# SingleRust/single-algebra

Hardware: AMD Instinct MI355X
Metric: sparse_pca_fit_transform_algorithmic_throughput (higher is better)
Workload: dtype f32

## Files before the change

single-algebra_amd/csrc/tiled_build.hip:

```cpp
#include <algorithm>
#include <cmath>
#include <cstdio>
#include <cstdlib>
#include <cstring>
#include <vector>

#include <rocprim/rocprim.hpp>

#include "kernels.h"
#include "quad_format.h"
#include "spmm_dq.h"

namespace sapca {
namespace k {

namespace {

__device__ __forceinline__ void divmod_small(int c, int d, float inv, int& q, int& r) {
  q = (int)((float)c * inv);
  r = c - q * d;
  if (r < 0) { r += d; --q; }
  if (r >= d) { r -= d; ++q; }
}

__global__ void __launch_bounds__(256)
tile_hist_kernel(const int64_t* __restrict__ ptr, const int32_t* __restrict__ idx, int64_t rows, int nct, float inv_nct,
                 int32_t* __restrict__ seg) {
  extern __shared__ uint32_t hist_all[];
  const int wave = threadIdx.x / WAVE, lane = threadIdx.x & (WAVE - 1);
  uint32_t* hist = hist_all + (size_t)wave * nct;
  for (int64_t r = (int64_t)blockIdx.x * 4 + wave; r < rows; r += (int64_t)gridDim.x * 4) {
    for (int t = lane; t < nct; t += WAVE) hist[t] = 0;
    __builtin_amdgcn_wave_barrier();
    const int64_t e0 = ptr[r], e1 = ptr[r + 1];
    for (int64_t eb = e0 + lane; eb < e1; eb += 8 * WAVE) {
      int c[8];
#pragma unroll
      for (int u = 0; u < 8; ++u) c[u] = eb + u * WAVE < e1 ? idx[eb + u * WAVE] : -1;
#pragma unroll
      for (int u = 0; u < 8; ++u)
        if (c[u] >= 0) {
          int q, t;
          divmod_small(c[u], nct, inv_nct, q, t);
          atomicAdd(&hist[t], 1u);
        }
    }
    __builtin_amdgcn_wave_barrier();
    uint32_t carry = 0;
    int32_t* out = seg + r * (nct + 1);
    for (int t0 = 0; t0 < nct; t0 += WAVE) {
      const int t = t0 + lane;
      const uint32_t v = t < nct ? hist[t] : 0u;
      uint32_t x = v;
#pragma unroll
      for (int off = 1; off < WAVE; off <<= 1) {
        const uint32_t y = __shfl_up(x, off);
        if (lane >= off) x += y;
      }
      if (t < nct) out[t] = (int32_t)(carry + x - v);
      carry += __shfl(x, WAVE - 1);
    }
    if (lane == 0) out[nct] = (int32_t)carry;
    __builtin_amdgcn_wave_barrier();
  }
}

constexpr int QC_TILES = 8;
__global__ void __launch_bounds__(Q_BLOCK_QUADS)
quad_count_kernel(const int32_t* __restrict__ seg, const int32_t* __restrict__ blk_row0, const uint32_t* __restrict__ perm,
                  int nct, uint16_t* __restrict__ steps, uint32_t* __restrict__ quad_off, uint32_t* __restrict__ wave_off,
                  int64_t* __restrict__ chunk_size, const uint16_t* __restrict__ cnt16 = nullptr, int64_t cnt_stride = 0,
                  int64_t* __restrict__ raw_size = nullptr) {
  __shared__ uint32_t scan[Q_BLOCK_QUADS];
  __shared__ uint32_t wave_total[Q_BLOCK_QUADS / WAVE], raw_part[Q_BLOCK_QUADS / WAVE];
  const int groups = (nct + QC_TILES - 1) / QC_TILES;
  const int rb = blockIdx.x / groups, ct0 = (blockIdx.x % groups) * QC_TILES;
  const int row0 = blk_row0[rb], nrows = blk_row0[rb + 1] - row0;
  const int nquads = (nrows + 3) / 4;
  const int q = threadIdx.x, lane = q & (WAVE - 1);
  int len[4][QC_TILES];
#pragma unroll
  for (int g = 0; g < 4; ++g) {
    const int lr = 4 * q + g;
    const bool have = lr < nrows;
    const int64_t r = have ? (perm ? (int64_t)perm[row0 + lr] : (int64_t)row0 + lr) : 0;
    if (cnt16) {
#pragma unroll
      for (int j = 0; j < QC_TILES; ++j) len[g][j] = (have && ct0 + j < nct) ? (int)cnt16[(int64_t)(ct0 + j) * cnt_stride + r] : 0;
    } else {
      int bound[QC_TILES + 1];
#pragma unroll
      for (int j = 0; j <= QC_TILES; ++j) bound[j] = (have && ct0 + j <= nct) ? seg[r * (nct + 1) + ct0 + j] : 0;
#pragma unroll
      for (int j = 0; j < QC_TILES; ++j) len[g][j] = (have && ct0 + j < nct) ? bound[j + 1] - bound[j] : 0;
    }
  }
#pragma unroll
  for (int j = 0; j < QC_TILES; ++j) {
    const int ct = ct0 + j;
    if (ct >= nct) break;
    const int64_t chunk = (int64_t)rb * nct + ct;
    const int longest = max(max(len[0][j], len[1][j]), max(len[2][j], len[3][j]));
    int raw = len[0][j] + len[1][j] + len[2][j] + len[3][j];
    const int qmax = q_steps(longest);
    const uint32_t padded = (uint32_t)qmax * 4u;
    steps[chunk * Q_BLOCK_QUADS + q] = (uint16_t)qmax;
    uint32_t inc = padded;
#pragma unroll
    for (int off = 1; off < WAVE; off <<= 1) {
      const uint32_t y = __shfl_up(inc, off);
      if (lane >= off) inc += y;
    }
#pragma unroll
    for (int off = WAVE / 2; off > 0; off >>= 1) raw += __shfl_xor(raw, off);
    __syncthreads();
    if (lane == WAVE - 1) wave_total[q / WAVE] = inc;
    if (lane == 0) raw_part[q / WAVE] = (uint32_t)raw;
    __syncthreads();
    for (int w = 0; w < q / WAVE; ++w) inc += wave_total[w];
    scan[q] = inc;
    __syncthreads();
    if (quad_off && q < nquads) quad_off[((int64_t)rb * Q_BLOCK_QUADS + q) * nct + ct] = inc - padded;
    if (q < QWAVES) {
      const int first_quad = q_first(q, nquads);
      wave_off[chunk * QWAVES + q] = first_quad > 0 ? scan[first_quad - 1] : 0u;
    }
    if (q == Q_BLOCK_QUADS - 1) {
      chunk_size[chunk] = inc;
      if (raw_size) {
        uint32_t total = 0;
        for (int w = 0; w < Q_BLOCK_QUADS / WAVE; ++w) total += raw_part[w];
        raw_size[chunk] = total;
      }
    }
  }
}

template <typename VT>
__global__ void __launch_bounds__(256)
quad_fill_kernel(const int64_t* __restrict__ ptr, const int32_t* __restrict__ idx, const VT* __restrict__ val,
                 int64_t rows, const int32_t* __restrict__ blk_row0, const uint32_t* __restrict__ perm, int nrb, int nct,
                 float inv_nct, int ldp_bytes, const int64_t* __restrict__ chunk_off, const uint32_t* __restrict__ quad_off,
                 typename EntOf<VT>::type* __restrict__ ent) {
  typedef typename EntOf<VT>::type E;
  extern __shared__ uint32_t cnt_all[];
  const int wave = threadIdx.x / WAVE, lane = threadIdx.x & (WAVE - 1);
  uint32_t* cnt = cnt_all + (size_t)wave * nct;
  const int64_t sp = (int64_t)blockIdx.x * 4 + wave;
  if (sp >= rows) return;
  const int64_t r = perm ? (int64_t)perm[sp] : sp;
  int lo = 0, hi = nrb;
  while (hi - lo > 1) {
    const int mid = (lo + hi) >> 1;
    if ((int64_t)blk_row0[mid] <= sp) lo = mid; else hi = mid;
  }
  const int rb = lo;
  const int lr = (int)(sp - blk_row0[rb]);
  const int qd = lr >> 2;
  const uint32_t g = (uint32_t)(lr & 3);
  const int64_t* __restrict__ coff = chunk_off + (int64_t)rb * nct;
  const uint32_t* __restrict__ qoff = quad_off + ((int64_t)rb * Q_BLOCK_QUADS + qd) * nct;
  const int64_t block_base = coff[0];
  for (int t = lane; t < nct; t += WAVE) cnt[t] = (uint32_t)(coff[t] - block_base) + qoff[t] + g;
  __builtin_amdgcn_wave_barrier();
  const int64_t e0 = ptr[r], e1 = ptr[r + 1];
  E* __restrict__ out = ent + block_base;
  for (int64_t eb = e0; eb < e1; eb += 8 * WAVE) {
    int c[8];
    VT v[8];
#pragma unroll
    for (int u = 0; u < 8; ++u) {
      const int64_t e = eb + u * WAVE + lane;
      c[u] = e < e1 ? idx[e] : -1;
      v[u] = e < e1 ? val[e] : (VT)0;
    }
#pragma unroll
    for (int u = 0; u < 8; ++u) {
      if (c[u] >= 0) {
        int i, t;
        divmod_small(c[u], nct, inv_nct, i, t);
        E x = E();
        x.off = (uint32_t)i * (uint32_t)ldp_bytes;
        x.val = v[u];
        out[atomicAdd(&cnt[t], 4u)] = x;
      }
      __builtin_amdgcn_wave_barrier();
    }
  }
}

constexpr int QF_CAP_MIN = 4096, QF_CAP_MAX = 6144;
template <typename VT>
__device__ __forceinline__ void quad_fill_staged_one(int qi, uint32_t* qf_lds, const int64_t* __restrict__ ptr, const int32_t* __restrict__ idx,
                                                     const VT* __restrict__ val, const int32_t* __restrict__ seg,
                                                     const int32_t* __restrict__ blk_row0, const uint32_t* __restrict__ perm, int nct, int cap,
                                                     float inv_nct, int ldp_bytes, const int64_t* __restrict__ chunk_off,
                                                     const uint32_t* __restrict__ quad_off, typename EntOf<VT>::type* __restrict__ ent) {
  typedef typename EntOf<VT>::type E;
  constexpr int EW = (int)sizeof(E) / 4;
  E* stage = reinterpret_cast<E*>(qf_lds);
  int64_t* gofs = reinterpret_cast<int64_t*>(qf_lds + EW * cap);
  uint32_t* lofs = qf_lds + EW * cap + 2 * nct;
  uint32_t* cnt_all = lofs + nct + 1;
  const int rb = qi / Q_BLOCK_QUADS, qd = qi % Q_BLOCK_QUADS;
  const int row0 = blk_row0[rb], nrows = blk_row0[rb + 1] - row0;
  if (4 * qd >= nrows) return;
  const int wave = threadIdx.x / WAVE, lane = threadIdx.x & (WAVE - 1);
  const int qrows = min(4, nrows - 4 * qd);
  const int64_t s0 = (int64_t)row0 + 4 * qd;
  int64_t rowof[4];
#pragma unroll
  for (int g = 0; g < 4; ++g) rowof[g] = g < qrows ? (perm ? (int64_t)perm[s0 + g] : s0 + g) : 0;
  const int64_t* __restrict__ coff = chunk_off + (int64_t)rb * nct;
  const uint32_t* __restrict__ qoff = quad_off + ((int64_t)rb * Q_BLOCK_QUADS + qd) * nct;
  for (int t = threadIdx.x; t < nct; t += 256) {
    int mx = 0;
    for (int g = 0; g < qrows; ++g) {
      const int32_t* sg = seg + rowof[g] * (nct + 1);
      mx = max(mx, sg[t + 1] - sg[t]);
    }
    lofs[t + 1] = (uint32_t)q_steps(mx) * 4u;
    gofs[t] = coff[t] + (int64_t)qoff[t];
    for (int g = 0; g < 4; ++g) cnt_all[g * nct + t] = 0;
  }
  if (threadIdx.x == 0) lofs[0] = 0;
  __syncthreads();
  if (wave == 0) {
    uint32_t carry = 0;
    for (int t0 = 0; t0 < nct; t0 += WAVE) {
      const int t = t0 + lane;
      const uint32_t v = t < nct ? lofs[t + 1] : 0u;
      uint32_t x = v;
#pragma unroll
      for (int off = 1; off < WAVE; off <<= 1) {
        const uint32_t y = __shfl_up(x, off);
        if (lane >= off) x += y;
      }
      if (t < nct) lofs[t + 1] = carry + x;
      carry += __shfl(x, WAVE - 1);
    }
  }
  __syncthreads();
  const uint32_t total = lofs[nct];
  const bool staged = total <= (uint32_t)cap;
  if (staged) {
    uint64_t* z = reinterpret_cast<uint64_t*>(stage);
    for (uint32_t i = threadIdx.x; i < total * (EW / 2); i += 256) z[i] = 0;
  } else {
    if (wave < qrows) {
      const int32_t* sg = seg + rowof[wave] * (nct + 1);
      for (int t = lane; t < nct; t += WAVE) {
        const uint32_t steps = (lofs[t + 1] - lofs[t]) / 4u;
        E* dst = ent + gofs[t];
        for (uint32_t k = (uint32_t)(sg[t + 1] - sg[t]); k < steps; ++k) dst[k * 4u + wave] = E();
      }
    } else {
      for (int t = lane; t < nct; t += WAVE) {
        const uint32_t steps = (lofs[t + 1] - lofs[t]) / 4u;
        E* dst = ent + gofs[t];
        for (uint32_t k = 0; k < steps; ++k) dst[k * 4u + wave] = E();
      }
    }
  }
  __syncthreads();
  if (wave < qrows) {
    const int64_t r = rowof[wave];
    const int64_t e0 = ptr[r], e1 = ptr[r + 1];
    uint32_t* cnt = cnt_all + (size_t)wave * nct;
    for (int64_t eb = e0; eb < e1; eb += 8 * WAVE) {
      int c[8];
      VT v[8];
#pragma unroll
      for (int u = 0; u < 8; ++u) {
        const int64_t e = eb + u * WAVE + lane;
        c[u] = e < e1 ? idx[e] : -1;
        v[u] = e < e1 ? val[e] : (VT)0;
      }
#pragma unroll
      for (int u = 0; u < 8; ++u) {
        if (c[u] >= 0) {
          int i, t;
          divmod_small(c[u], nct, inv_nct, i, t);
          E x = E();
          x.off = (uint32_t)i * (uint32_t)ldp_bytes;
          x.val = v[u];
          const uint32_t k = atomicAdd(&cnt[t], 1u);
          if (staged) stage[lofs[t] + k * 4u + (uint32_t)wave] = x;
          else ent[gofs[t] + k * 4u + (uint32_t)wave] = x;
        }
        __builtin_amdgcn_wave_barrier();
      }
    }
  }
  if (!staged) return;
  __syncthreads();
  for (int t = wave; t < nct; t += 4) {
    const uint32_t lo = lofs[t], n = lofs[t + 1] - lo;
    E* dst = ent + gofs[t];
    for (uint32_t j = lane; j < n; j += WAVE) dst[j] = stage[lo + j];
  }
}

template <typename VT>
__global__ void __launch_bounds__(256)
quad_fill_staged_kernel(const int64_t* __restrict__ ptr, const int32_t* __restrict__ idx, const VT* __restrict__ val,
                        const int32_t* __restrict__ seg, const int32_t* __restrict__ blk_row0,
                        const uint32_t* __restrict__ perm, int nct, int cap, float inv_nct,
                        int ldp_bytes, const int64_t* __restrict__ chunk_off, const uint32_t* __restrict__ quad_off,
                        typename EntOf<VT>::type* __restrict__ ent, int nquads_all) {
  extern __shared__ __attribute__((aligned(16))) uint32_t qf_lds[];
  for (int qi = blockIdx.x; qi < nquads_all; qi += gridDim.x) {
    quad_fill_staged_one<VT>(qi, qf_lds, ptr, idx, val, seg, blk_row0, perm, nct, cap, inv_nct, ldp_bytes, chunk_off, quad_off, ent);
    __syncthreads();
  }
}

__global__ void tile_index_mod_kernel(const int64_t* __restrict__ ptr, const int32_t* __restrict__ idx,
                                      const uint64_t* __restrict__ packed, int64_t rows, int nct, float inv_nct,
                                      int32_t* __restrict__ seg) {
  const int64_t total = rows * (int64_t)(nct + 1);
  int64_t o = (int64_t)blockIdx.x * blockDim.x + threadIdx.x;
  const int64_t stride = (int64_t)gridDim.x * blockDim.x;
  for (; o < total; o += stride) {
    const int64_t r = o / (nct + 1);
    const int t = (int)(o - r * (nct + 1));
    const int64_t e0 = ptr[r], e1 = ptr[r + 1];
    int64_t lo = e0, hi = e1;
    while (lo < hi) {
      const int64_t mid = (lo + hi) >> 1;
      int q, tm;
      divmod_small(packed ? (int)(packed[mid] >> 32) : idx[mid], nct, inv_nct, q, tm);
      if (tm < t) lo = mid + 1; else hi = mid;
    }
    seg[o] = (int32_t)(lo - e0);
  }
}

__global__ void at_stats_index_kernel(const int64_t* __restrict__ ptr, const uint64_t* __restrict__ packed, int64_t rows,
                                      int nct, float inv_nct, double* __restrict__ sum, double* __restrict__ sumsq,
                                      int32_t* __restrict__ seg) {
  const int lane = threadIdx.x & (WAVE - 1);
  const int64_t wave = ((int64_t)blockIdx.x * blockDim.x + threadIdx.x) / WAVE;
  const int64_t nwaves = (int64_t)gridDim.x * blockDim.x / WAVE;
  for (int64_t r = wave; r < rows; r += nwaves) {
    const int64_t e0 = ptr[r], e1 = ptr[r + 1];
    int32_t* sg = seg + r * (nct + 1);
    double a = 0, b = 0;
    int carry = -1;
    for (int64_t eb = e0; eb < e1; eb += WAVE) {
      const int64_t e = eb + lane;
      const bool valid = e < e1;
      int t = nct;
      if (valid) {
        const uint64_t pv = packed[e];
        const double v = (double)__uint_as_float((uint32_t)pv);
        a += v;
        b += v * v;
        int q;
        divmod_small((int)(pv >> 32), nct, inv_nct, q, t);
      }
      int tprev = __shfl_up(t, 1);
      if (lane == 0) tprev = carry;
      if (valid || e == e1)
        for (int tt = tprev + 1; tt <= t; ++tt) sg[tt] = (int32_t)(e - e0);
      carry = __shfl(t, WAVE - 1);
    }
    if (((e1 - e0) & (WAVE - 1)) == 0)
      for (int tt = carry + 1 + lane; tt <= nct; tt += WAVE) sg[tt] = (int32_t)(e1 - e0);
#pragma unroll
    for (int off = WAVE / 2; off > 0; off >>= 1) {
      a += __shfl_xor(a, off);
      b += __shfl_xor(b, off);
    }
    if (lane == 0) {
      sum[r] = a;
      if (sumsq) sumsq[r] = b;
    }
  }
}

__global__ void row_len_iota_kernel(const int64_t* __restrict__ ptr, int64_t rows, uint32_t* __restrict__ len,
                                    uint32_t* __restrict__ iota) {
  const int64_t r = (int64_t)blockIdx.x * blockDim.x + threadIdx.x;
  if (r < rows) {
    len[r] = (uint32_t)(ptr[r + 1] - ptr[r]);
    iota[r] = (uint32_t)r;
  }
}

__global__ void __launch_bounds__(256)
natural_quad_slots_kernel(const int64_t* __restrict__ ptr, int64_t rows, unsigned long long* __restrict__ out) {
  __shared__ unsigned long long red[4];
  unsigned long long acc = 0;
  const int64_t nq = (rows + 3) / 4;
  for (int64_t qd = (int64_t)blockIdx.x * blockDim.x + threadIdx.x; qd < nq; qd += (int64_t)gridDim.x * blockDim.x) {
    int64_t mx = 0;
    for (int g = 0; g < 4 && 4 * qd + g < rows; ++g) mx = max(mx, ptr[4 * qd + g + 1] - ptr[4 * qd + g]);
    acc += (unsigned long long)(4 * mx);
  }
#pragma unroll
  for (int off = WAVE / 2; off > 0; off >>= 1) acc += __shfl_xor(acc, off);
  if ((threadIdx.x & (WAVE - 1)) == 0) red[threadIdx.x / WAVE] = acc;
  __syncthreads();
  if (threadIdx.x == 0) atomicAdd(out, red[0] + red[1] + red[2] + red[3]);
}

template <bool SEG_LDS, typename VT = float>
__global__ void __launch_bounds__(256)
quad_fill_runs_kernel(const int64_t* __restrict__ ptr, const int32_t* __restrict__ idx, const VT* __restrict__ val,
                      const uint64_t* __restrict__ packed, const int32_t* __restrict__ seg, const int32_t* __restrict__ blk_row0,
                      const uint32_t* __restrict__ perm, int nct, float inv_nct, int ldp_bytes,
                      const int64_t* __restrict__ chunk_off, const uint32_t* __restrict__ quad_off,
                      typename EntOf<VT>::type* __restrict__ ent) {
  typedef typename EntOf<VT>::type Ent;
  extern __shared__ int32_t sg_lds[];
  const int rb = blockIdx.x / Q_BLOCK_QUADS, qd = blockIdx.x % Q_BLOCK_QUADS;
  const int row0 = blk_row0[rb], nrows = blk_row0[rb + 1] - row0;
  if (4 * qd >= nrows) return;
  const int wave = threadIdx.x / WAVE, lane = threadIdx.x & (WAVE - 1);
  const int qrows = min(4, nrows - 4 * qd);
  const int64_t s0q = (int64_t)row0 + 4 * qd;
  if (SEG_LDS) {
    for (int i = threadIdx.x; i < 4 * (nct + 1); i += 256) {
      const int g = i / (nct + 1);
      const int64_t rg = g < qrows ? (perm ? (int64_t)perm[s0q + g] : s0q + g) : 0;
      sg_lds[i] = g < qrows ? seg[rg * (nct + 1) + (i - g * (nct + 1))] : 0;
    }
    __syncthreads();
  }
  const int g = lane & 3, k0 = lane >> 2;
  const int64_t myrow = g < qrows ? (perm ? (int64_t)perm[s0q + g] : s0q + g) : -1;
  const int64_t base = myrow >= 0 ? ptr[myrow] : 0;
  const int32_t* mysg = SEG_LDS ? sg_lds + g * (nct + 1) : seg + (myrow >= 0 ? myrow : 0) * (nct + 1);
  const int64_t* __restrict__ coff = chunk_off + (int64_t)rb * nct;
  const uint32_t* __restrict__ qoff = quad_off + ((int64_t)rb * Q_BLOCK_QUADS + qd) * nct;
  int s_nx = 0, e_nx = 0;
  int64_t d_nx = 0;
  if (!SEG_LDS && wave < nct) {
    s_nx = myrow >= 0 ? mysg[wave] : 0;
    e_nx = myrow >= 0 ? mysg[wave + 1] : 0;
    d_nx = coff[wave] + qoff[wave];
  }
  for (int t = wave; t < nct; t += 4) {
    int s0, len;
    Ent* dst;
    if (SEG_LDS) {
      s0 = mysg[t];
      len = mysg[t + 1] - s0;
      dst = ent + coff[t] + qoff[t];
    } else {
      s0 = s_nx;
      len = e_nx - s_nx;
      dst = ent + d_nx;
      if (t + 4 < nct) {
        s_nx = myrow >= 0 ? mysg[t + 4] : 0;
        e_nx = myrow >= 0 ? mysg[t + 5] : 0;
        d_nx = coff[t + 4] + qoff[t + 4];
      }
    }
    int qmax = max(len, __shfl_xor(len, 1));
    qmax = q_steps(max(qmax, __shfl_xor(qmax, 2)));
    for (int k = k0; k < qmax; k += 16) {
      Ent x{};
      if (k < len) {
        const int64_t e = base + s0 + k;
        int c;
        if constexpr (sizeof(VT) == 4) {
          if (packed) {
            const uint64_t pv = packed[e];
            c = (int)(pv >> 32);
            x.val = __uint_as_float((uint32_t)pv);
          } else {
            c = idx[e];
            x.val = val[e];
          }
        } else {
          c = idx[e];
          x.val = val[e];
        }
        int i, tm;
        divmod_small(c, nct, inv_nct, i, tm);
        x.off = (uint32_t)i * (uint32_t)ldp_bytes;
      }
      dst[k * 4 + g] = x;
    }
  }
}

template <int PER, bool HAS_B>
__global__ void __launch_bounds__(1024)
small_scan_kernel(int64_t* __restrict__ a, int64_t* __restrict__ b, int64_t count, int64_t* __restrict__ out_max_total) {
  __shared__ int64_t wsum[2][16], wmax[16];
  const int tid = threadIdx.x, lane = tid & (WAVE - 1), wave = tid / WAVE;
  int64_t carry_a = 0, carry_b = 0, m = 0;
  for (int64_t base = 0; base < count; base += 1024 * PER) {
    const int64_t lo = min(count, base + (int64_t)tid * PER), hi = min(count, lo + PER);
    int64_t sa = 0, sb = 0, mx = 0;
    int64_t ra_[PER], rb_[HAS_B ? PER : 1];
#pragma unroll
    for (int u = 0; u < PER; ++u) {
      ra_[u] = lo + u < hi ? a[lo + u] : 0;
      if constexpr (HAS_B) rb_[u] = lo + u < hi ? b[lo + u] : 0;
    }
#pragma unroll
    for (int u = 0; u < PER; ++u) {
      sa += ra_[u];
      mx = max(mx, ra_[u]);
      if constexpr (HAS_B) sb += rb_[u];
    }
    int64_t ia = sa, ib = sb;
#pragma unroll
    for (int off = 1; off < WAVE; off <<= 1) {
      const int64_t ya = __shfl_up(ia, off), yb = __shfl_up(ib, off);
      if (lane >= off) { ia += ya; ib += yb; }
    }
#pragma unroll
    for (int off = WAVE / 2; off > 0; off >>= 1) mx = max(mx, __shfl_xor(mx, off));
    __syncthreads();
    if (lane == WAVE - 1) { wsum[0][wave] = ia; wsum[1][wave] = ib; }
    if (lane == 0) wmax[wave] = mx;
    __syncthreads();
    int64_t ra = carry_a + ia - sa, rb = carry_b + ib - sb, ta = 0, tb = 0;
#pragma unroll 2
    for (int w = 0; w < 16; ++w) {
      if (w < wave) { ra += wsum[0][w]; rb += wsum[1][w]; }
      ta += wsum[0][w];
      tb += wsum[1][w];
      m = max(m, wmax[w]);
    }
    carry_a += ta;
    carry_b += tb;
#pragma unroll
    for (int u = 0; u < PER; ++u) {
      if (lo + u < hi) {
        a[lo + u] = ra;
        if constexpr (HAS_B) b[lo + u] = rb;
      }
      ra += ra_[u];
      if constexpr (HAS_B) rb += rb_[u];
    }
  }
  if (tid == 0) {
    a[count] = carry_a;
    if (HAS_B && b) b[count] = carry_b;
    if (out_max_total) { out_max_total[0] = m; out_max_total[1] = carry_a; }
  }
}

void launch_small_scan(int64_t* a, int64_t* b, int64_t count, int64_t* out_max_total, hipStream_t s) {
  const int64_t per = (count + 1023) / 1024;
  if (b && per <= 8) hipLaunchKernelGGL((small_scan_kernel<8, true>), dim3(1), dim3(1024), 0, s, a, b, count, out_max_total);
  else if (b) hipLaunchKernelGGL((small_scan_kernel<16, true>), dim3(1), dim3(1024), 0, s, a, b, count, out_max_total);
  else hipLaunchKernelGGL((small_scan_kernel<24, false>), dim3(1), dim3(1024), 0, s, a, b, count, out_max_total);
}

constexpr int ATD_MAX_COLS = 65536;
constexpr int ATD_THREADS = 1024;
constexpr int ATD_MASK_WORDS = 10;

constexpr int ATD_HIST_THREADS = 512;
constexpr int ATD_HIST_THREADS_WIDE = 1024;

__global__ void __launch_bounds__(ATD_HIST_THREADS_WIDE)
atd_hist_kernel(const int64_t* __restrict__ ptr, const int32_t* __restrict__ idx, int64_t m, int nct, int tc, int64_t n2,
                uint16_t* __restrict__ cnt16, float blk_scale, int nrb, uint32_t* __restrict__ bnd, int64_t* __restrict__ disorder,
                unsigned long long* __restrict__ slots_to_clear) {
  if (blockIdx.x == 0 && threadIdx.x == 0 && slots_to_clear) *slots_to_clear = 0ull;
  extern __shared__ uint32_t atd_h32[];
  const int t = blockIdx.x;
  const int nw = (int)(n2 / 2);
  const int nthreads = (int)blockDim.x, nwaves = nthreads / WAVE;
  for (int i = threadIdx.x; i < nw; i += nthreads) atd_h32[i] = 0u;
  __syncthreads();
  const int wave = threadIdx.x / WAVE, lane = threadIdx.x & (WAVE - 1);
  int64_t r = (int64_t)t + (int64_t)wave * nct;
  int64_t e0 = (wave < tc && r < m) ? ptr[r] : 0, e1 = (wave < tc && r < m) ? ptr[r + 1] : 0;
  for (int i = wave; i < tc; i += nwaves) {
    if (r >= m) {
      if (bnd)
        for (int j = lane; j <= nrb; j += WAVE) bnd[((int64_t)t * tc + i) * (nrb + 1) + j] = 0u;
      continue;
    }
    const int64_t rn = r + (int64_t)nwaves * nct;
    const bool more = i + nwaves < tc && rn < m;
    const int64_t n0 = more ? ptr[rn] : 0, n1 = more ? ptr[rn + 1] : 0;
    int lastb = -1;
    uint32_t* __restrict__ bnd_row = bnd ? bnd + ((int64_t)t * tc + i) * (nrb + 1) : nullptr;
    const int64_t row_e0 = e0;
    for (int64_t base = e0; base < e1; base += 8 * WAVE) {
      const int64_t eb = base + lane;
      int c[8];
#pragma unroll
      for (int u = 0; u < 8; ++u) c[u] = eb + u * WAVE < e1 ? idx[eb + u * WAVE] : -1;
      if (bnd) {
#pragma unroll
        for (int u = 0; u < 8; ++u) {
          const bool valid = c[u] >= 0;
          const unsigned long long valids = __ballot(valid);
          if (valids == 0ull) break;
          const int b = (int)((float)max(c[u], 0) * blk_scale);
          const int up = __builtin_amdgcn_update_dpp(0, b, 0x138, 0xf, 0xf, false);
          const int prev = lane == 0 ? lastb : up;
          if (valid && b != prev)
            for (int j = prev + 1; j <= b; ++j) bnd_row[j] = (uint32_t)(eb + u * WAVE - row_e0);
          if (valid && b < prev) *disorder = 1;
          lastb = __builtin_amdgcn_readlane(b, __builtin_popcountll(valids) - 1);
        }
      }
#pragma unroll
      for (int u = 0; u < 8; ++u)
        if (c[u] >= 0) atomicAdd(&atd_h32[c[u] >> 1], 1u << (16 * (c[u] & 1)));
    }
    if (bnd)
      for (int j = lastb + 1 + lane; j <= nrb; j += WAVE) bnd_row[j] = (uint32_t)(e1 - row_e0);
    r = rn;
    e0 = n0;
    e1 = n1;
  }
  __syncthreads();
  uint32_t* out = reinterpret_cast<uint32_t*>(cnt16 + (int64_t)t * n2);
  for (int i = threadIdx.x; i < nw; i += nthreads) out[i] = atd_h32[i];
}

__global__ void __launch_bounds__(1024)
atd_rowlen_kernel(const uint16_t* __restrict__ cnt16, int64_t n, int64_t n2, int nct, int64_t* __restrict__ len,
                  unsigned long long* __restrict__ natural_slots) {
  __shared__ uint32_t part[16][64];
  const int lane = threadIdx.x & 63, grp = threadIdx.x >> 6;
  const int64_t c = (int64_t)blockIdx.x * 64 + lane;
  const int per = (nct + 15) / 16;
  uint32_t a = 0;
  if (c < n) {
    const int t1 = min(nct, (grp + 1) * per);
    int t = grp * per;
    for (; t + 8 <= t1; t += 8) {
      uint32_t v[8];
#pragma unroll
      for (int u = 0; u < 8; ++u) v[u] = cnt16[(int64_t)(t + u) * n2 + c];
#pragma unroll
      for (int u = 0; u < 8; ++u) a += v[u];
    }
    for (; t < t1; ++t) a += cnt16[(int64_t)t * n2 + c];
  }
  part[grp][lane] = a;
  __syncthreads();
  if (grp == 0) {
    int64_t total = 0;
    if (c < n)
      for (int g = 0; g < 16; ++g) total += part[g][lane];
    if (c <= n) len[c] = total;
    if (natural_slots) {
      int64_t mx = max(total, __shfl_xor(total, 1));
      mx = max(mx, __shfl_xor(mx, 2));
      unsigned long long acc = (lane & 3) == 0 ? (unsigned long long)(4 * mx) : 0ull;
#pragma unroll
      for (int off = WAVE / 2; off > 0; off >>= 1) acc += __shfl_xor(acc, off);
      if (lane == 0 && acc) atomicAdd(natural_slots, acc);
    }
  }
}

__global__ void atd_colmap_kernel(const int32_t* __restrict__ blk, int nrb, const uint32_t* __restrict__ perm, int64_t rows,
                                  uint32_t* __restrict__ colmap) {
  const int64_t sp = (int64_t)blockIdx.x * blockDim.x + threadIdx.x;
  if (sp >= rows) return;
  int lo = 0, hi = nrb;
  while (lo + 1 < hi) {
    const int mid = (lo + hi) >> 1;
    if ((int64_t)blk[mid] <= sp) lo = mid; else hi = mid;
  }
  const int64_t row = perm ? (int64_t)perm[sp] : sp;
  colmap[row] = ((uint32_t)lo << 10) | (uint32_t)(sp - blk[lo]);
}

__global__ void __launch_bounds__(256)
atd_scatter_kernel(const int64_t* __restrict__ ptr, const int32_t* __restrict__ idx, const float* __restrict__ val, int64_t m, int nct,
                   int tc, const uint32_t* __restrict__ colmap, const int64_t* __restrict__ bucket_off, uint32_t* __restrict__ cursor,
                   uint2* __restrict__ bucket) {
  const int lane = threadIdx.x & (WAVE - 1);
  const int xcd = blockIdx.x & 7;
  const int64_t wave = (int64_t)(blockIdx.x >> 3) * (blockDim.x / WAVE) + threadIdx.x / WAVE;
  const int64_t nwaves = (int64_t)(gridDim.x >> 3) * (blockDim.x / WAVE);
  const int tiles_x = (nct - xcd + 7) / 8;
  const int64_t items = (int64_t)tiles_x * tc;
  constexpr int UB = 10;
  for (int64_t item = wave; item < items; item += nwaves) {
    const int i = (int)(item / tiles_x), t = xcd + 8 * (int)(item - (int64_t)i * tiles_x);
    const int64_t r = (int64_t)t + (int64_t)i * nct;
    if (r >= m) continue;
    const int64_t e1 = ptr[r + 1];
    for (int64_t eb = ptr[r]; eb < e1; eb += UB * WAVE) {
      int cc[UB];
      uint32_t cmv[UB];
      float vv[UB];
      int64_t base[UB];
      int mine[UB];
#pragma unroll
      for (int u = 0; u < UB; ++u) {
        const int64_t e = eb + u * WAVE + lane;
        cc[u] = e < e1 ? idx[e] : -1;
        vv[u] = e < e1 ? val[e] : 0.f;
      }
#pragma unroll
      for (int u = 0; u < UB; ++u) cmv[u] = cc[u] >= 0 ? colmap[cc[u]] : 0xffffffffu;
#pragma unroll
      for (int u = 0; u < UB; ++u) {
        const uint32_t rb = cmv[u] >> 10;
        const uint32_t prev = __shfl_up(rb, 1);
        const bool valid = cc[u] >= 0;
        const bool leader = valid && (lane == 0 || rb != prev);
        const unsigned long long leaders = __ballot(leader), valids = __ballot(valid);
        const unsigned long long upto = leaders & ((2ull << lane) - 1ull);
        mine[u] = upto ? 63 - __builtin_clzll(upto) : 0;
        base[u] = 0;
        if (leader) {
          const unsigned long long above = leaders & ~((2ull << lane) - 1ull);
          const int next = above ? __builtin_ctzll(above) : __builtin_popcountll(valids);
          const int64_t b = (int64_t)rb * nct + t;
          base[u] = bucket_off[b] + (int64_t)atomicAdd(&cursor[b], (uint32_t)(next - lane));
        }
      }
#pragma unroll
      for (int u = 0; u < UB; ++u) {
        const int64_t b0 = __shfl(base[u], mine[u]);
        if (cc[u] >= 0)
          bucket[b0 + (lane - mine[u])] = make_uint2(((cmv[u] & 1023u) << 9) | (uint32_t)i, __float_as_uint(vv[u]));
      }
    }
  }
}

constexpr int ATD_STAGE_ENT = 4096;

template <bool GATHER>
__global__ void __launch_bounds__(ATD_THREADS, 8)
atd_fill_kernel(const uint2* __restrict__ bucket, const int64_t* __restrict__ bucket_off, const int32_t* __restrict__ blk_row0,
                const uint32_t* __restrict__ perm, int nct, int ldp_bytes, const int64_t* __restrict__ chunk_off,
                const uint32_t* __restrict__ quad_off, const uint16_t* __restrict__ steps, Ent* __restrict__ ent,
                double* __restrict__ psum, double* __restrict__ psq, int64_t n,
                const int32_t* __restrict__ a_idx, const float* __restrict__ a_val, const uint32_t* __restrict__ bnd,
                const int64_t* __restrict__ a_ptr, int64_t a_rows, int tc, int nrb_all) {
  constexpr int MASK_WORDS_ALL = QBLOCK_ROWS * ATD_MASK_WORDS;
  __shared__ __attribute__((aligned(16))) uint32_t pool[MASK_WORDS_ALL + 2 * ATD_STAGE_ENT];
  uint32_t* mask = pool;
  Ent* stage = reinterpret_cast<Ent*>(pool + MASK_WORDS_ALL);
  __shared__ uint32_t qoff_s[Q_BLOCK_QUADS + 1];
  __shared__ uint32_t wtot[Q_BLOCK_QUADS / WAVE];
  __shared__ uint16_t len_s[QBLOCK_ROWS];
  __shared__ int64_t run_lo[GATHER ? 32 * ATD_MASK_WORDS : 1];
  __shared__ uint32_t run_pre[GATHER ? 32 * ATD_MASK_WORDS + 1 : 1];
  __shared__ uint32_t rtot[GATHER ? 32 * ATD_MASK_WORDS / WAVE : 1];
  int rb, t;
  if constexpr (GATHER) {
    const int xcd = blockIdx.x & 7, j = blockIdx.x >> 3;
    t = xcd + 8 * (j / nrb_all);
    rb = j % nrb_all;
    if (t >= nct) return;
  } else {
    rb = (int)(blockIdx.x / nct);
    t = (int)(blockIdx.x % nct);
  }
  const int64_t chunk = (int64_t)rb * nct + t;
  const int row0 = blk_row0[rb], nrows = blk_row0[rb + 1] - row0;
  const int nquads = (nrows + 3) / 4;
  for (int i = threadIdx.x; i < QBLOCK_ROWS * ATD_MASK_WORDS; i += ATD_THREADS) mask[i] = 0u;
  if (threadIdx.x < Q_BLOCK_QUADS) {
    const int q = threadIdx.x, lane = q & (WAVE - 1);
    const uint32_t sz = q < nquads ? 4u * (uint32_t)steps[chunk * Q_BLOCK_QUADS + q] : 0u;
    uint32_t inc = sz;
#pragma unroll
    for (int off = 1; off < WAVE; off <<= 1) {
      const uint32_t y = __shfl_up(inc, off);
      if (lane >= off) inc += y;
    }
    qoff_s[q + 1] = inc;
    if (lane == WAVE - 1) wtot[q / WAVE] = inc;
  }
  if constexpr (GATHER) {
    if (threadIdx.x < 32 * ATD_MASK_WORDS) {
      const int i = threadIdx.x, lane = i & (WAVE - 1);
      const uint32_t* br = bnd + ((int64_t)t * tc + i) * (nrb_all + 1) + rb;
      const int64_t arow = (int64_t)t + (int64_t)i * nct;
      const int64_t e0 = (i < tc && arow < a_rows) ? a_ptr[arow] : 0;
      const int64_t lo = i < tc ? e0 + br[0] : 0;
      const int64_t hi = i < tc ? e0 + br[1] : 0;
      run_lo[i] = lo;
      uint32_t inc = hi > lo ? (uint32_t)(hi - lo) : 0u;
#pragma unroll
      for (int off = 1; off < WAVE; off <<= 1) {
        const uint32_t y = __shfl_up(inc, off);
        if (lane >= off) inc += y;
      }
      run_pre[i + 1] = inc;
      if (lane == WAVE - 1) rtot[i / WAVE] = inc;
    }
  }
  __syncthreads();
  if (threadIdx.x < Q_BLOCK_QUADS) {
    uint32_t add = 0;
    for (int w = 0; w < (int)threadIdx.x / WAVE; ++w) add += wtot[w];
    qoff_s[threadIdx.x + 1] += add;
    if (threadIdx.x == 0) qoff_s[0] = 0u;
  }
  if constexpr (GATHER) {
    if (threadIdx.x < 32 * ATD_MASK_WORDS) {
      uint32_t add = 0;
      for (int w = 0; w < (int)threadIdx.x / WAVE; ++w) add += rtot[w];
      run_pre[threadIdx.x + 1] += add;
      if (threadIdx.x == 0) run_pre[0] = 0u;
    }
  }
  __syncthreads();
  const int64_t b0 = GATHER ? 0 : bucket_off[chunk];
  const int64_t b1 = GATHER ? (int64_t)(uint32_t)__builtin_amdgcn_readfirstlane((int)run_pre[32 * ATD_MASK_WORDS]) : bucket_off[chunk + 1];
  constexpr int HOLD = 10;
  uint16_t* row_of = reinterpret_cast<uint16_t*>(stage);
  if constexpr (GATHER) {
    if (threadIdx.x < 3 * 32 * ATD_MASK_WORDS) {
      const uint32_t i = threadIdx.x / 3u;
      const uint32_t k1 = min(run_pre[i + 1], (uint32_t)(HOLD * ATD_THREADS));
      for (uint32_t k = run_pre[i] + threadIdx.x % 3u; k < k1; k += 3u) row_of[k] = (uint16_t)i;
    }
    __syncthreads();
  }
  auto fetch = [&](int64_t f, bool tabled) -> uint2 {
    if constexpr (GATHER) {
      int lo = 0;
      if (tabled) {
        lo = row_of[f];
      } else {
        int hi = 32 * ATD_MASK_WORDS - 1;
        while (lo < hi) {
          const int mid = (lo + hi + 1) >> 1;
          if ((int64_t)run_pre[mid] <= f) lo = mid; else hi = mid - 1;
        }
      }
      const int64_t e = run_lo[lo] + (f - (int64_t)run_pre[lo]);
      return make_uint2(((uint32_t)(a_idx[e] - row0) << 9) | (uint32_t)lo, __float_as_uint(a_val[e]));
    } else {
      return bucket[f];
    }
  };
  Ent* dst = ent + chunk_off[chunk];
  uint2 kv[HOLD];
#pragma unroll
  for (int u = 0; u < HOLD; ++u) {
    const int64_t e = b0 + threadIdx.x + (int64_t)u * ATD_THREADS;
    kv[u] = e < b1 ? fetch(e, true) : make_uint2(0xffffffffu, 0u);
  }
#pragma unroll
  for (int u = 0; u < HOLD; ++u)
    if (kv[u].x != 0xffffffffu) {
      const uint32_t slot = kv[u].x >> 9, i = kv[u].x & 511u;
      atomicOr(&mask[slot * ATD_MASK_WORDS + (i >> 5)], 1u << (i & 31u));
    }
  for (int64_t e = b0 + threadIdx.x + (int64_t)HOLD * ATD_THREADS; e < b1; e += ATD_THREADS) {
    const uint32_t key = fetch(e, false).x;
    const uint32_t slot = key >> 9, i = key & 511u;
    atomicOr(&mask[slot * ATD_MASK_WORDS + (i >> 5)], 1u << (i & 31u));
  }
  __syncthreads();
  const bool held = b1 - b0 <= (int64_t)HOLD * ATD_THREADS;
  uint16_t* pre = reinterpret_cast<uint16_t*>(stage);
  for (int slot = threadIdx.x; slot < QBLOCK_ROWS; slot += ATD_THREADS) {
    uint32_t run = 0;
#pragma unroll
    for (int w = 0; w < ATD_MASK_WORDS; ++w) {
      if (held) pre[slot * ATD_MASK_WORDS + w] = (uint16_t)run;
      run += __builtin_popcount(mask[slot * ATD_MASK_WORDS + w]);
    }
    len_s[slot] = (uint16_t)run;
  }
  __syncthreads();
  auto rank_of = [&](uint32_t slot, uint32_t i) {
    const uint32_t* mk = mask + slot * ATD_MASK_WORDS;
    uint32_t rank = __builtin_popcount(mk[i >> 5] & ((1u << (i & 31u)) - 1u));
    if (held) return rank + (uint32_t)pre[slot * ATD_MASK_WORDS + (i >> 5)];
    for (uint32_t w = 0; w < (i >> 5); ++w) rank += __builtin_popcount(mk[w]);
    return rank;
  };
#pragma unroll
  for (int u = 0; u < HOLD; ++u) {
    if (kv[u].x != 0xffffffffu) {
      const uint32_t slot = kv[u].x >> 9, i = kv[u].x & 511u;
      kv[u].x = (qoff_s[slot >> 2] + rank_of(slot, i) * 4u + (slot & 3u)) | (i << 23);
    }
    asm volatile("" ::: "memory");
  }
  const uint32_t HALF = held ? (uint32_t)(MASK_WORDS_ALL / 2 + ATD_STAGE_ENT) / 2u : (uint32_t)ATD_STAGE_ENT / 2u;
  Ent* const image = held ? reinterpret_cast<Ent*>(pool) : stage;
  __syncthreads();
  auto row_len = [&](int slot) { return (int)len_s[slot]; };
  int half = 0;
  for (int q0 = 0; q0 < nquads; half ^= 1) {
    int q1 = q0 + 1;
    {
      int lo = q0 + 1, hi = nquads;
      while (lo < hi) {
        const int mid = (lo + hi + 1) >> 1;
        if (qoff_s[mid] - qoff_s[q0] <= HALF) lo = mid; else hi = mid - 1;
      }
      q1 = __builtin_amdgcn_readfirstlane(lo);
    }
    Ent* st = image + (half ? HALF : 0u);
    const uint32_t o0 = (uint32_t)__builtin_amdgcn_readfirstlane((int)qoff_s[q0]);
    const uint32_t size = (uint32_t)__builtin_amdgcn_readfirstlane((int)qoff_s[q1]) - o0;
    for (int slot = 4 * q0 + (int)threadIdx.x; slot < 4 * q1; slot += ATD_THREADS) {
      const uint32_t qo = qoff_s[slot >> 2], nsteps = (qoff_s[(slot >> 2) + 1] - qo) / 4u;
      const uint32_t o = qo - o0 + (uint32_t)(slot & 3);
#pragma clang loop vectorize(disable) unroll(disable)
      for (uint32_t k = slot < nrows ? (uint32_t)row_len(slot) : 0u; k < nsteps; ++k) st[o + 4u * k] = Ent{0u, 0.f};
    }
    auto place = [&](uint32_t slot, uint32_t i, uint32_t rank, uint32_t vbits) {
      const int q = (int)(slot >> 2);
      if (q < q0 || q >= q1) return;
      Ent x;
      x.off = i * (uint32_t)ldp_bytes;
      x.val = __uint_as_float(vbits);
      st[qoff_s[q] - o0 + rank * 4u + (slot & 3u)] = x;
    };
#pragma unroll
// ... 587 lines not shown
```

Before: 1350.

## Software-pipeline index loads in histogram kernels with double-buffered row windows

Rewrites tile_hist_kernel and atd_hist_kernel so each wave loads a 12-wide window of column indices into registers for the next chunk (or next row) while it processes the current one. Two register buffers alternate, and row pointers are prefetched two rows ahead. Loads are clamped to stay in bounds instead of predicated, which removes per-element branches. This is meant to hide global-memory latency behind LDS atomics, at the cost of higher register pressure and more complex control flow.

New measurement: 1351, median of 2. No clear change (+0.0%).

```diff
diff --git a/single-algebra_amd/csrc/tiled_build.hip b/single-algebra_amd/csrc/tiled_build.hip
--- a/single-algebra_amd/csrc/tiled_build.hip
+++ b/single-algebra_amd/csrc/tiled_build.hip
@@ -23,28 +23,64 @@
   if (r >= d) { r -= d; ++q; }
 }
 
+constexpr int ROW_WIN = 12;
+constexpr int ROW_WIN_ENTRIES = ROW_WIN * WAVE;
+struct Window { int64_t first; int n; };
+__device__ __forceinline__ Window window_at(int64_t base, int64_t end, int entries) {
+  const int n = (int)max((int64_t)0, min(end - base, (int64_t)entries));
+  return {n > 0 ? base : 0, n};
+}
+__device__ __forceinline__ bool in_window(int n, int lane, int u) { return lane + u * WAVE < n; }
+template <typename T>
+__device__ __forceinline__ T window_load(const T* __restrict__ first, const Window& w, int lane, int u) {
+  const uint32_t byte = (uint32_t)max(min(lane + u * WAVE, w.n - 1), 0) * (uint32_t)sizeof(T);
+  return *reinterpret_cast<const T*>(reinterpret_cast<const char*>(first) + byte);
+}
+template <typename T>
+__device__ __forceinline__ void arrived(T x) { asm volatile("" ::"v"(x)); }
+__device__ __forceinline__ int load_index_window(int (&c)[ROW_WIN], const int32_t* __restrict__ idx, int64_t base, int64_t end, int lane) {
+  const Window w = window_at(base, end, ROW_WIN_ENTRIES);
+  const int32_t* __restrict__ p = idx + w.first;
+#pragma unroll
+  for (int u = 0; u < ROW_WIN; ++u) c[u] = window_load(p, w, lane, u);
+  return w.n;
+}
+
 __global__ void __launch_bounds__(256)
 tile_hist_kernel(const int64_t* __restrict__ ptr, const int32_t* __restrict__ idx, int64_t rows, int nct, float inv_nct,
                  int32_t* __restrict__ seg) {
   extern __shared__ uint32_t hist_all[];
-  const int wave = threadIdx.x / WAVE, lane = threadIdx.x & (WAVE - 1);
+  const int wave = __builtin_amdgcn_readfirstlane(threadIdx.x / WAVE), lane = threadIdx.x & (WAVE - 1);
   uint32_t* hist = hist_all + (size_t)wave * nct;
-  for (int64_t r = (int64_t)blockIdx.x * 4 + wave; r < rows; r += (int64_t)gridDim.x * 4) {
-    for (int t = lane; t < nct; t += WAVE) hist[t] = 0;
-    __builtin_amdgcn_wave_barrier();
-    const int64_t e0 = ptr[r], e1 = ptr[r + 1];
-    for (int64_t eb = e0 + lane; eb < e1; eb += 8 * WAVE) {
-      int c[8];
-#pragma unroll
-      for (int u = 0; u < 8; ++u) c[u] = eb + u * WAVE < e1 ? idx[eb + u * WAVE] : -1;
-#pragma unroll
-      for (int u = 0; u < 8; ++u)
-        if (c[u] >= 0) {
-          int q, t;
-          divmod_small(c[u], nct, inv_nct, q, t);
-          atomicAdd(&hist[t], 1u);
-        }
-    }
+  const int64_t stride = (int64_t)gridDim.x * 4;
+  int64_t r = (int64_t)blockIdx.x * 4 + wave;
+  if (r >= rows) return;
+  int64_t e0 = ptr[r], e1 = ptr[r + 1], n0 = 0, n1 = 0;
+  if (r + stride < rows) { n0 = ptr[r + stride]; n1 = ptr[r + stride + 1]; }
+  int ca[ROW_WIN], cb[ROW_WIN];
+  int na = load_index_window(ca, idx, e0, e1, lane), nb = 0;
+  int64_t wb = e0;
+  auto step = [&](const int (&c)[ROW_WIN], int n, int (&cn)[ROW_WIN], int& nn) {
+    const bool last = r < rows && wb + ROW_WIN_ENTRIES >= e1;
+    int64_t nn0 = 0, nn1 = 0;
+    if (last && r + 2 * stride < rows) { nn0 = ptr[r + 2 * stride]; nn1 = ptr[r + 2 * stride + 1]; }
+    const int64_t next = last ? n0 : wb + ROW_WIN_ENTRIES;
+    nn = load_index_window(cn, idx, next, last ? n1 : e1, lane);
+    if (wb == e0) {
+      for (int t = lane; t < nct; t += WAVE) hist[t] = 0;
+      __builtin_amdgcn_wave_barrier();
+    }
+#pragma unroll
+    for (int u = 0; u < ROW_WIN; ++u) {
+      arrived(c[u]);
+      if (in_window(n, lane, u)) {
+        int q, t;
+        divmod_small(c[u], nct, inv_nct, q, t);
+        atomicAdd(&hist[t], 1u);
+      }
+    }
+    wb = next;
+    if (!last) return;
     __builtin_amdgcn_wave_barrier();
     uint32_t carry = 0;
     int32_t* out = seg + r * (nct + 1);
@@ -62,7 +98,13 @@
     }
     if (lane == 0) out[nct] = (int32_t)carry;
     __builtin_amdgcn_wave_barrier();
-  }
+    r += stride;
+    e0 = n0; e1 = n1; n0 = nn0; n1 = nn1;
+  };
+  do {
+    step(ca, na, cb, nb);
+    step(cb, nb, ca, na);
+  } while (r < rows);
 }
 
 constexpr int QC_TILES = 8;
@@ -570,53 +612,62 @@
   const int t = blockIdx.x;
   const int nw = (int)(n2 / 2);
   const int nthreads = (int)blockDim.x, nwaves = nthreads / WAVE;
-  for (int i = threadIdx.x; i < nw; i += nthreads) atd_h32[i] = 0u;
+  const int wave = __builtin_amdgcn_readfirstlane(threadIdx.x / WAVE), lane = threadIdx.x & (WAVE - 1);
+  const int64_t rstride = (int64_t)nwaves * nct;
+  int i = wave;
+  int64_t r = (int64_t)t + (int64_t)wave * nct;
+  int64_t e0 = 0, e1 = 0, n0 = 0, n1 = 0;
+  if (i < tc && r < m) { e0 = ptr[r]; e1 = ptr[r + 1]; }
+  if (i + nwaves < tc && r + rstride < m) { n0 = ptr[r + rstride]; n1 = ptr[r + rstride + 1]; }
+  int ca[ROW_WIN], cb[ROW_WIN];
+  int na = load_index_window(ca, idx, e0, e1, lane), nb = 0;
+  for (int j = threadIdx.x; j < nw; j += nthreads) atd_h32[j] = 0u;
   __syncthreads();
-  const int wave = threadIdx.x / WAVE, lane = threadIdx.x & (WAVE - 1);
-  int64_t r = (int64_t)t + (int64_t)wave * nct;
-  int64_t e0 = (wave < tc && r < m) ? ptr[r] : 0, e1 = (wave < tc && r < m) ? ptr[r + 1] : 0;
-  for (int i = wave; i < tc; i += nwaves) {
-    if (r >= m) {
-      if (bnd)
-        for (int j = lane; j <= nrb; j += WAVE) bnd[((int64_t)t * tc + i) * (nrb + 1) + j] = 0u;
-      continue;
-    }
-    const int64_t rn = r + (int64_t)nwaves * nct;
-    const bool more = i + nwaves < tc && rn < m;
-    const int64_t n0 = more ? ptr[rn] : 0, n1 = more ? ptr[rn + 1] : 0;
-    int lastb = -1;
+  int64_t wb = e0;
+  int lastb = -1;
+  auto step = [&](const int (&c)[ROW_WIN], int n, int (&cn)[ROW_WIN], int& nn) {
+    const bool last = i < tc && r < m && wb + ROW_WIN_ENTRIES >= e1;
+    int64_t nn0 = 0, nn1 = 0;
+    if (last && i + 2 * nwaves < tc && r + 2 * rstride < m) { nn0 = ptr[r + 2 * rstride]; nn1 = ptr[r + 2 * rstride + 1]; }
+    const int64_t next = last ? n0 : wb + ROW_WIN_ENTRIES;
+    nn = load_index_window(cn, idx, next, last ? n1 : e1, lane);
     uint32_t* __restrict__ bnd_row = bnd ? bnd + ((int64_t)t * tc + i) * (nrb + 1) : nullptr;
-    const int64_t row_e0 = e0;
-    for (int64_t base = e0; base < e1; base += 8 * WAVE) {
-      const int64_t eb = base + lane;
-      int c[8];
-#pragma unroll
-      for (int u = 0; u < 8; ++u) c[u] = eb + u * WAVE < e1 ? idx[eb + u * WAVE] : -1;
-      if (bnd) {
-#pragma unroll
-        for (int u = 0; u < 8; ++u) {
-          const bool valid = c[u] >= 0;
-          const unsigned long long valids = __ballot(valid);
-          if (valids == 0ull) break;
-          const int b = (int)((float)max(c[u], 0) * blk_scale);
-          const int up = __builtin_amdgcn_update_dpp(0, b, 0x138, 0xf, 0xf, false);
-          const int prev = lane == 0 ? lastb : up;
-          if (valid && b != prev)
-            for (int j = prev + 1; j <= b; ++j) bnd_row[j] = (uint32_t)(eb + u * WAVE - row_e0);
-          if (valid && b < prev) *disorder = 1;
-          lastb = __builtin_amdgcn_readlane(b, __builtin_popcountll(valids) - 1);
-        }
-      }
-#pragma unroll
-      for (int u = 0; u < 8; ++u)
-        if (c[u] >= 0) atomicAdd(&atd_h32[c[u] >> 1], 1u << (16 * (c[u] & 1)));
-    }
+    const uint32_t at0 = (uint32_t)(wb - e0) + (uint32_t)lane;
+    if (bnd) {
+#pragma unroll
+      for (int u = 0; u < ROW_WIN; ++u) {
+        if (u * WAVE >= n) break;
+        const bool valid = in_window(n, lane, u);
+        const int b = (int)((float)max(c[u], 0) * blk_scale);
+        const int up = __builtin_amdgcn_update_dpp(0, b, 0x138, 0xf, 0xf, false);
+        const int prev = lane == 0 ? lastb : up;
+        if (valid && b != prev)
+          for (int j = prev + 1; j <= b; ++j) bnd_row[j] = at0 + u * WAVE;
+        if (valid && b < prev) *disorder = 1;
+        lastb = __builtin_amdgcn_readlane(b, min(n - u * WAVE, WAVE) - 1);
+      }
+    }
+#pragma unroll
+    for (int u = 0; u < ROW_WIN; ++u) {
+      arrived(c[u]);
+      if (in_window(n, lane, u)) atomicAdd(&atd_h32[c[u] >> 1], 1u << (16 * (c[u] & 1)));
+    }
+    wb = next;
+    if (!last) return;
     if (bnd)
-      for (int j = lastb + 1 + lane; j <= nrb; j += WAVE) bnd_row[j] = (uint32_t)(e1 - row_e0);
-    r = rn;
-    e0 = n0;
-    e1 = n1;
-  }
+      for (int j = lastb + 1 + lane; j <= nrb; j += WAVE) bnd_row[j] = (uint32_t)(e1 - e0);
+    lastb = -1;
+    i += nwaves;
+    r += rstride;
+    e0 = n0; e1 = n1; n0 = nn0; n1 = nn1;
+  };
+  while (i < tc && r < m) {
+    step(ca, na, cb, nb);
+    step(cb, nb, ca, na);
+  }
+  if (bnd)
+    for (; i < tc; i += nwaves)
+      for (int j = lane; j <= nrb; j += WAVE) bnd[((int64_t)t * tc + i) * (nrb + 1) + j] = 0u;
   __syncthreads();
   uint32_t* out = reinterpret_cast<uint32_t*>(cnt16 + (int64_t)t * n2);
   for (int i = threadIdx.x; i < nw; i += nthreads) out[i] = atd_h32[i];
```
